# Bazs/structure_from_motion

Measured on AMD Instinct MI355X. Metric: correspondence-evals/s (matches x hypotheses), higher is better.
Workload: dtype f64 (+ conservative f16/bf16 matrix-pipe reject filter)

## Files before the change

structure_from_motion_amd/csrc/sfm_score.hip:

```cpp
#include <hip/hip_runtime.h>
#include <math.h>
#include <stdint.h>
#include <stdlib.h>

#include <algorithm>
#include <atomic>

#include "sfm_common.h"
#include "sfm_math.h"
#include "sfm_score_ws.h"
#include "sfm_score_matrix.h"

namespace {

using namespace sfmws;
using sfmhost::check_launch;
using sfmhost::fail;
using sfmhost::grid_for;
using sfmhost::grid_stride;

constexpr int kHypPerWave = 4;
#ifndef SFM_WAVE_STAMPS
#define SFM_WAVE_STAMPS 0
#endif
// ... 237 lines not shown
        c[k] = 0;
    }
    const int limit = min(n, kEstimatePoints);
    for (int i = lane; i < limit; i += kWave) {
        const float4 p = pts32[i];
#pragma unroll
        for (int k = 0; k < HPW; ++k) {
            if (ONE_SIDED) {
                const unsigned long long rej = reject_mask_one_sided(f[k], p.x, p.y, p.z, p.w);
                c[k] += (int)((~rej >> lane) & 1ull);
            } else {
                c[k] += filter_rejects(f[k], T, p.x, p.y, p.z, p.w) ? 0 : 1;
            }
        }
    }
#pragma unroll
    for (int k = 0; k < HPW; ++k) {
        const int total = sfm::wave_sum(c[k]);
        const int h = h0 + k;
        if (h < h_count && lane == 0) estimate[b * (int64_t)h_count + h] = total * 16;
    }
}

SFM_DEVICE int cost_class(int estimate) {
    if (estimate <= 0) return kClasses - 1;
    const unsigned e = (unsigned)min(estimate, 16384);
    const int lg = 31 - __builtin_clz(e);
    const int sixteenth = lg >= 4 ? (int)((e >> (lg - 4)) & 15u) : (int)((e << (4 - lg)) & 15u);
    return 16 * (14 - lg) + (15 - sixteenth);
}
static_assert(kEstimatePoints == 1024 && kClasses == 16 * 15 + 1, "cost_class: estimates up to 2^14 in 240 classes + one for zero");

__global__ __launch_bounds__(256) void score_class_count_kernel(const int32_t* __restrict__ estimate, int h_count,
                                                                int32_t* __restrict__ buckets) {
    static_assert(kClasses <= 256, "one thread per class");
    __shared__ int block_count[256];
    const int64_t b = blockIdx.y;
    const int h = blockIdx.x * blockDim.x + threadIdx.x;
    block_count[threadIdx.x] = 0;
    __syncthreads();
    if (h < h_count) atomicAdd(&block_count[cost_class(estimate[b * (int64_t)h_count + h])], 1);
    __syncthreads();
    if (threadIdx.x < kClasses && block_count[threadIdx.x] != 0)
        atomicAdd(buckets + b * kBuckets + threadIdx.x * kClassStride, block_count[threadIdx.x]);
}

__global__ __launch_bounds__(256) void score_class_scan_kernel(int32_t* __restrict__ buckets, int64_t batch) {
    __shared__ int scan[256];
    const int64_t b = blockIdx.x;
    const int c = threadIdx.x;
    const int own = c < kClasses ? buckets[b * kBuckets + c * kClassStride] : 0;
    scan[c] = own;
    __syncthreads();
#pragma unroll
// ... 435 lines not shown

void launch_matrix_setup(const sfmhost::ScorePlan& p, const sfmhost::ScoreArrays& io, unsigned* select_state) {
    hipLaunchKernelGGL(matrixscore::matrix_setup_kernel, dim3(p.matrix.setup_blocks, (unsigned)p.batch), dim3(256), 0, io.stream,
                       (const Corr*)io.corr, (int)p.n, p.a_scale, p.partial, p.buckets, io.cnt, (int)p.h_count, select_state);
}

int launch_matrix(const sfmhost::ScorePlan& p, const sfmhost::ScoreArrays& io, bool tables_ready, bool fold_in_selection) {
    using namespace matrixscore;
    static_assert(kBlocks * 2 * 16 == 96, "sfm_score_ws.h sizes the tables: 3 blocks");
    const auto& m = p.matrix;
    const unsigned pairs = (unsigned)p.batch;
    if (!tables_ready) {
        launch_matrix_setup(p, io, nullptr);
        hipLaunchKernelGGL(matrix_tables_kernel, dim3((unsigned)m.table_blocks + grid_for(2 * p.h_count, 256), pairs), dim3(256), 0,
                           io.stream, (const Corr*)io.corr, (int)p.n, p.a_scale, (const float4*)p.partial, (int)m.setup_blocks, p.table,
                           m.table_blocks, io.E, (int)p.h_count, p.hyp_table, io.S, p.thr, p.fix);
    }
    const int32_t* order_arg = nullptr;
    if (p.use_order) {
        hipLaunchKernelGGL((score_sed_matrix_kernel<true, 0, false>), dim3(m.prepass_blocks), dim3(256), 0, io.stream, (const Corr*)io.corr,
                           (const uint4*)p.hyp_table, (const uint4*)p.table, (int)p.n, io.E, (int)p.h_count, p.thr, (const int32_t*)nullptr,
                           io.cnt, io.s1, io.s2, m.prepass_units, m.prepass_steps, (unsigned char*)nullptr, (const unsigned char*)nullptr,
                           (int)p.batch, m.prepass_blocks_per_pair, (int32_t*)nullptr, p.record, p.per_unit, p.ws.units,
                           (const int32_t*)nullptr, 0);
        const dim3 per_hyp(grid_for(p.h_count, 256), pairs);
        hipLaunchKernelGGL(score_class_count_kernel, per_hyp, dim3(256), 0, io.stream, io.cnt, (int)p.h_count, p.buckets);
        hipLaunchKernelGGL(score_class_scan_scatter_kernel, per_hyp, dim3(256), 0, io.stream, io.cnt, (int)p.h_count, p.buckets, p.order,
                           m.wide_from_min, m.wide_from_max);
        const int rc = check_launch("score order kernels");
        if (rc != SFM_OK) return rc;
        order_arg = p.order;
    }
    if (p.opt.timing_before) (void)hipEventRecord((hipEvent_t)p.opt.timing_before, io.stream);
    const auto scoring_kernel = m.wide_waves ? score_sed_matrix_kernel<false, SFM_MATRIX_MASK_GROUP_WIDE, true>
                                : p.batch > 1 ? score_sed_matrix_kernel<false, SFM_MATRIX_MASK_GROUP_BATCH, false>
                                              : score_sed_matrix_kernel<false, SFM_MATRIX_MASK_GROUP_SINGLE, false>;
    hipLaunchKernelGGL(scoring_kernel, dim3(m.scoring_blocks), dim3(256), 0, io.stream, (const Corr*)io.corr, (const uint4*)p.hyp_table,
                       (const uint4*)p.table, (int)p.n, io.E, (int)p.h_count, p.thr, order_arg, io.cnt, io.s1, io.s2, p.ws.units, p.per_unit,
                       p.split, (const unsigned char*)p.fix, (int)p.batch, m.blocks_per_pair, m.persistent ? p.buckets + kTicketWords : nullptr,
                       p.record, 0, 0, m.wide_waves ? p.buckets + kWideFromWord : nullptr, m.wide_from_max);
    if (p.opt.timing_after) (void)hipEventRecord((hipEvent_t)p.opt.timing_after, io.stream);
    if (!fold_in_selection && p.ws.units > 1)
        hipLaunchKernelGGL(matrix_fold_kernel, dim3(grid_stride(p.h_count, 256, 1024), pairs), dim3(256), 0, io.stream, p.split,
                           (const unsigned char*)p.fix, p.ws.units, (int)p.h_count, io.cnt, io.s1, io.s2);
    return check_launch("score_sed_matrix_kernel");
}

constexpr sfm_score_options kBuiltinOptions = SFM_SCORE_OPTIONS_DEFAULT;
std::atomic<const sfm_score_options*> g_default_options{&kBuiltinOptions};

bool valid_options(const sfm_score_options& o) {
    return (o.kernel == SFM_SCORE_KERNEL_AUTO || o.kernel == SFM_SCORE_KERNEL_FILTERED || o.kernel == SFM_SCORE_KERNEL_MATRIX) &&
           (o.hyps_per_wave == 0 || o.hyps_per_wave == 1 || o.hyps_per_wave == 2 || o.hyps_per_wave == 4) && o.split >= -1 &&
           o.order >= -1 && o.order <= 1 && o.one_sided >= -1 && o.one_sided <= 1 && o.xcd_map >= -1 && o.xcd_map <= 1 &&
           o.block_sync >= -1 && o.persistent >= -1 && o.persistent <= 1;
}

bool load_options(const sfm_score_options* given, sfm_score_options* out) {
    *out = given ? *given : *g_default_options.load(std::memory_order_acquire);
    return valid_options(*out);
}

int refuse(const char* fn, const char* what) {
    snprintf(sfmhost::error_buffer(), sfmhost::kErrorBytes, "%s: %s", fn, what);
    return SFM_EINVAL;
}
constexpr const char* kBeyondOneLaunch = "size exceeds what one launch covers (2^31-1 blocks, 2^32-1 threads in x; 65535 in y/z)";

bool use_matrix_kernel(int64_t n, int64_t h_count, int64_t batch, const sfm_score_options& opt) {
    const int matrix_env = opt.kernel == SFM_SCORE_KERNEL_MATRIX ? 1 : opt.kernel == SFM_SCORE_KERNEL_FILTERED ? 0 : -1;
    const int64_t waves32_all = (h_count + matrixscore::kHyps - 1) / matrixscore::kHyps * batch;
    const bool matrix_fits = n <= matrixscore::kMaxPoints &&
                             sfmhost::grid_fits((int64_t)grid_for((h_count + 31) / 32, 256 / kWave) * ((batch + 7) / 8 * 8), 1, 256);
    const bool matrix_pays = batch == 1 ? (n >= 4000 && h_count >= 2048 && (double)n * (double)h_count >= 3.5e8)
                                        : (n >= 8192 && h_count >= 1024 && waves32_all >= 6144 &&
                                           (double)n * (double)h_count * (double)batch >= 5e8);
    return matrix_fits && (matrix_env > 0 || (matrix_env < 0 && matrix_pays));
}

constexpr int kRecordRangesPerWave = 2;

int plan_launches(const char* fn, sfmhost::ScorePlan* p) {
    const int64_t n = p->n, h_count = p->h_count, batch = p->batch;
    const sfm_score_options& opt = p->opt;
    int hpw = kHypPerWave;
    if (opt.hyps_per_wave != 0) {
        hpw = opt.hyps_per_wave;
    } else {
        while (hpw > 1 && (h_count + hpw - 1) / hpw * batch < 5120) hpw /= 2;
    }
    if (!sfmhost::grid_fits((h_count + hpw - 1) / hpw, 256 / kWave, 256, batch)) return refuse(fn, kBeyondOneLaunch);
    if (!sfmhost::grid_fits(h_count, 256, 256, batch)) return refuse(fn, "the ordering pre-pass exceeds what one launch covers");
    const int64_t waves = (h_count + kHypPerWave - 1) / kHypPerWave;
    const int order_env = opt.order;
    const bool use_order = order_env >= 0 ? order_env != 0 : (waves * batch <= 12 * 5120 && n >= 8192);
    const bool matrix = use_matrix_kernel(n, h_count, batch, opt);
    const bool one_sided = opt.one_sided != 0;
    p->a_scale = matrix ? matrixscore::scale_for(p->thr) : (one_sided ? one_sided_scale(p->thr) : 1.0);
    const int split_env = opt.split;
    p->small.hpw = opt.hyps_per_wave != 0 ? opt.hyps_per_wave : (h_count + 1) / 2 >= 5120 ? 2 : 1;
    p->small.blocks = grid_for((h_count + p->small.hpw - 1) / p->small.hpw, 256 / kWave);
    p->small.sync_every = opt.block_sync >= 0 ? opt.block_sync : (p->small.hpw == 1 && n >= 4096 ? 2 : 0);
    p->small.prep_blocks = (int)((n + kPrepPoints - 1) / kPrepPoints);
// ... 55 lines not shown
                        steps_per_unit >= kReplaySteps && steps - (m_units - 1) * steps_per_unit >= kReplaySteps;
    p->ws = WsPlan{true, m_units, record};
    p->use_order = matrix_order;
    p->per_unit = steps_per_unit;
    auto& m = p->matrix;
    m.setup_blocks = grid_stride(n, 1024, matrixscore::kSetupBlocks);
    m.table_blocks = (int)((matrixscore::table_steps(n) + 3) / 4);
    m.wide_waves = batch == 1 && matrix_order && h_count >= SFM_MATRIX_WIDE_MIN_HYPOTHESES;
    m.wide_from_min = m.wide_waves ? SFM_MATRIX_WIDE_FROM : 0;
    m.wide_from_max = m.wide_waves ? matrixscore::kWideFromMax : 0;
    using matrixscore::kHyps;
    const int64_t scoring_waves = m.wide_waves ? m.wide_from_max / kHyps + (h_count + 2 * kHyps - 1) / (2 * kHyps) : waves32;
    const unsigned blocks = grid_for(scoring_waves, 256 / kWave);
    const unsigned blocks_of_32 = grid_for(waves32, 256 / kWave);
    const unsigned groups = batch > 1 ? (unsigned)((batch + 7) / 8 * 8) : 1u;
    m.blocks_per_pair = batch > 1 ? (int)blocks * m_units : 0;
    m.persistent = batch == 1 && opt.persistent > 0;
    m.scoring_blocks = blocks * groups * (unsigned)m_units;
    const int e_steps = matrixscore::estimate_steps(n);
    m.prepass_units = record ? (batch == 1 ? std::max(1, m_units / kRecordRangesPerWave) : 1) : (batch == 1 && e_steps >= 128 ? 4 : 1);
    m.prepass_steps = record ? kReplaySteps : e_steps / m.prepass_units;
    m.prepass_blocks = blocks_of_32 * groups * (unsigned)m.prepass_units;
    m.prepass_blocks_per_pair = batch > 1 ? (int)blocks_of_32 * m.prepass_units : 0;
    return SFM_OK;
}

int compute_units() {
    static std::atomic<int> cached[64];
    int device = 0;
    if (hipGetDevice(&device) != hipSuccess || device < 0 || device >= 64) return 256;
    int cus = cached[device].load(std::memory_order_relaxed);
    if (cus == 0) {
        if (hipDeviceGetAttribute(&cus, hipDeviceAttributeMultiprocessorCount, device) != hipSuccess || cus <= 0) cus = 256;
        cached[device].store(cus, std::memory_order_relaxed);
    }
    return cus;
}

}

namespace sfmhost {

int plan_score(const char* fn, int64_t n, int64_t h_count, int64_t batch, double thr, const sfm_score_options* options,
               void* workspace, int64_t workspace_bytes, ScorePlan* plan) {
    *plan = ScorePlan{};
    plan->n = n;
// ... 216 lines not shown
```

structure_from_motion_amd/csrc/sfm_score_matrix.h:

```cpp
#pragma once

#ifndef SFM_MATRIX_OCC
#define SFM_MATRIX_OCC 4
#endif
#ifndef SFM_MATRIX_POPS
#define SFM_MATRIX_POPS 4
#endif
#ifndef SFM_MATRIX_MASK_GROUP_SINGLE
#define SFM_MATRIX_MASK_GROUP_SINGLE 4
#endif
#ifndef SFM_MATRIX_MASK_GROUP_WIDE
#define SFM_MATRIX_MASK_GROUP_WIDE 2
#endif
#ifndef SFM_MATRIX_MASK_GROUP_BATCH
#define SFM_MATRIX_MASK_GROUP_BATCH 2
#endif
#ifndef SFM_MATRIX_STATS
#define SFM_MATRIX_STATS 0
#endif

#include "sfm_matrix_tables.h"

namespace matrixscore {

#if SFM_MATRIX_STATS
__device__ unsigned long long g_matrix_stats[4];
// ... 17 lines not shown
#endif
constexpr int kWideOcc = 3;
#ifndef SFM_MATRIX_WIDE_MIN_HYPOTHESES
#define SFM_MATRIX_WIDE_MIN_HYPOTHESES 8192
#endif
#ifndef SFM_MATRIX_WIDE_FROM
#define SFM_MATRIX_WIDE_FROM 4096
#endif
constexpr int kWideFromMax = 4 * SFM_MATRIX_WIDE_FROM;
static_assert(kWideFromMax % kHyps == 0, "waves of 32 cover the entries [0, kWideFromMax) exactly");
constexpr int kCap = SFM_MATRIX_CAP;
constexpr int kHigh = kCap - 4;
constexpr int kLow = 8;
constexpr int kPops = SFM_MATRIX_POPS;
#ifndef SFM_MATRIX_AHEAD
#define SFM_MATRIX_AHEAD 1
#endif
static_assert(SFM_MATRIX_AHEAD >= 1 && kHigh + 2 * (SFM_MATRIX_AHEAD + 1) - 1 <= kCap, "a group of kAhead + 1 steps (two entries each in a wide wave) must fit behind kHigh - 1 entries");
static_assert(SFM_MATRIX_AHEAD + 1 <= 4, "the point operand table is padded to a multiple of four steps");
constexpr int kAhead = SFM_MATRIX_AHEAD;
#ifndef SFM_MATRIX_ESTIMATE_AHEAD
#define SFM_MATRIX_ESTIMATE_AHEAD 1
#endif
static_assert(SFM_MATRIX_ESTIMATE_AHEAD == 1 || SFM_MATRIX_ESTIMATE_AHEAD == 3, "the recording pre-pass packs steps in pairs; the table is padded to four steps");
#ifndef SFM_MATRIX_ESTIMATE_STEPS
#define SFM_MATRIX_ESTIMATE_STEPS 128
#endif
constexpr int kEstimateSteps = SFM_MATRIX_ESTIMATE_STEPS;
constexpr int64_t kMaxPoints = sfmws::kMatrixMaxPoints;
constexpr int kMaxRangeSteps = 32768;
static_assert(kMaxPoints <= (int64_t)sfmws::kSplitMaxUnits * kMaxRangeSteps * kTile, "sixteen ranges of 2^15 steps cover the largest pair");

__host__ __device__ inline int estimate_steps(int64_t n) {
    const int64_t eighth = steps_of(n) / 8;
    return (int)(eighth < 32 ? 32 : eighth > kEstimateSteps ? kEstimateSteps : eighth);
}

__global__ __launch_bounds__(256) void matrix_prepare_kernel(const Corr* __restrict__ corr, int n, double c,
                                                            const unsigned char* __restrict__ ws, uint4* __restrict__ table) {
    const int64_t pair = blockIdx.y;
    const int t = (int)blockIdx.x * 4 + (int)(threadIdx.x / kWave);
    if (t >= (int)table_steps(n)) return;
    prepare_step(corr + pair * (int64_t)n, n, c, reinterpret_cast<const uint32_t*>(ws + 16 * pair),
                 table + pair * table_steps(n) * kBlocks * 64, t, (int)(threadIdx.x & (kWave - 1)));
}

__global__ __launch_bounds__(256) void matrix_hypothesis_kernel(const unsigned char* __restrict__ ws, const double* __restrict__ E,
// ... 194 lines not shown
    const f16x8 B1 = __builtin_bit_cast(f16x8, operands[1]);
    const bf16x8 B2 = __builtin_bit_cast(bf16x8, operands[2]);
    const uint4* __restrict__ operands_second = hyp_table + ((int64_t)h_second * 2 + half) * kBlocks;
    const f16x8 C0 = __builtin_bit_cast(f16x8, operands_second[0]);
    const f16x8 C1 = __builtin_bit_cast(f16x8, operands_second[1]);
    const bf16x8 C2 = __builtin_bit_cast(bf16x8, operands_second[2]);
    SFM_STAMP(1);

    int c = 0;
    unsigned head = 0, tail = 0, cur = 0;
    constexpr unsigned kSlotBytes = kWave * 4, kRingMask = (kCap - 1) * kSlotBytes;
    typedef __attribute__((address_space(3))) uint32_t lds_u32;
    const uint32_t queue_base = (uint32_t)(uintptr_t)(lds_u32*)my_queue;
    auto ring_slot = [&](unsigned counter) __attribute__((always_inline)) {
        return (lds_u32*)(uintptr_t)(queue_base | (counter & kRingMask));
    };
    unsigned cur_off = 0;
    double a1 = 0.0, a2 = 0.0;
#if SFM_MATRIX_STATS || SFM_MATRIX_STAMPS
    unsigned stat_rounds = 0, stat_pops = 0, stat_push_iterations = 0;
#endif

    const int steps_total = (int)steps_of(n);
    const bool recording = ESTIMATE && a.record != nullptr;
    const bool replaying = !ESTIMATE && a.record != nullptr;
    const int step_begin = units > 1 ? unit * (recording ? a.range_stride : steps_per_unit) : 0;
    const int64_t record_stride = sfmws::split_padded(h_count) * 2;
    uint4* const my_record = a.record == nullptr ? nullptr
        : reinterpret_cast<uint4*>(a.record) + (int64_t)unit * (kReplaySteps / 8) * record_stride + (int64_t)h * 2 + (WIDE ? 0 : half);
    const int step_end = units > 1 || ESTIMATE ? min(step_begin + steps_per_unit, steps_total) : steps_total;
    const int last_loadable = (int)table_steps(n) - 1;

    const sfm::SedGate gate = sfm::sed_gate(thr);
    const unsigned lane_off = (unsigned)((step_begin * kTile + (WIDE ? 0 : 16 * half) - 16) * (int)sizeof(Corr));
    auto round = [&]() __attribute__((always_inline)) {
        Corr p[kPops];
        bool active[kPops];
#pragma unroll
        for (int k = 0; k < kPops; ++k) {
            if ((cur == 0u) & (head != tail)) {
                const unsigned entry = *ring_slot(head);
                head += kSlotBytes;
                cur = entry & 0xffffu;
                cur_off = lane_off + ((entry >> 16) << (WIDE ? 9 : 10));
            }
            active[k] = cur != 0u;
            const unsigned lz = (unsigned)__builtin_clz(cur | 1u);
            cur &= ~(0x80000000u >> lz);
            const unsigned off = active[k] ? cur_off + (lz << 5) : 0u;
// ... 5 lines not shown
        for (int k = 0; k < kPops; ++k) stat_pops += active[k] ? 1u : 0u;
#endif
        auto evaluate = [&](int from, int to) __attribute__((always_inline)) {
#pragma unroll
            for (int k = from; k < to; ++k) {
                double sed;
                const bool ok = sfm::sed_inlier(e, p[k].xa, p[k].ya, p[k].xb, p[k].yb, gate, sed) && active[k];
                c += ok ? 1 : 0;
                const double kept = ok ? sed : 0.0;
                a1 += kept;
                a2 = fma(kept, kept, a2);
            }
        };
        if (MASK_GROUP > 0) {
#pragma unroll
            for (int g = 0; g < kPops; g += (MASK_GROUP > 0 ? MASK_GROUP : kPops))
                if (active[g]) evaluate(g, g + MASK_GROUP < kPops ? g + MASK_GROUP : kPops);
        } else {
            evaluate(0, kPops);
        }
    };

    unsigned survivors = 0;
    unsigned rec[4] = {0u, 0u, 0u, 0u}, rec_low = 0u;
    unsigned rec_upper[4] = {0u, 0u, 0u, 0u}, rec_upper_low = 0u;
    static_assert((kAhead + 1) % 2 == 0, "the recording pre-pass packs the steps of a loop group two to a dword");
    const int first_step = step_begin + (replaying ? kReplaySteps : 0);
    if (step_begin < step_end) {
        const uint4* __restrict__ src = table + lane;
        const unsigned lane_bytes = (unsigned)lane * 16u;
        const __amdgpu_buffer_rsrc_t table_rsrc = __builtin_amdgcn_make_buffer_rsrc(
            const_cast<uint4*>(table), (short)0, (int)(table_steps(n) * (int64_t)(kBlocks * 64 * 16)), 0x00020000);
        constexpr int kStages = (ESTIMATE ? SFM_MATRIX_ESTIMATE_AHEAD : kAhead) + 1;
        uint4 A[kStages][kBlocks];
#pragma unroll
        for (int a = 0; a < kStages; ++a) {
#pragma unroll
            for (int b = 0; b < kBlocks; ++b) A[a][b] = src[((size_t)min(first_step + a, last_loadable) * kBlocks + b) * 64];
            __builtin_amdgcn_sched_barrier(0);
        }
        if (replaying) {
            unsigned words[kReplaySteps / 2], words_upper[kReplaySteps / 2];
#pragma unroll
            for (int q = 0; q < kReplaySteps / 8; ++q) {
                const uint4 w = my_record[q * record_stride];
                words[4 * q] = w.x, words[4 * q + 1] = w.y, words[4 * q + 2] = w.z, words[4 * q + 3] = w.w;
                if (WIDE) {
                    const uint4 u = my_record[q * record_stride + 1];
                    words_upper[4 * q] = u.x, words_upper[4 * q + 1] = u.y, words_upper[4 * q + 2] = u.z, words_upper[4 * q + 3] = u.w;
// ... 40 lines not shown
                float16v r2 = {0, 0, 0, 0, 0, 0, 0, 0, 0, 0, 0, 0, 0, 0, 0, 0}, d2 = r2;
                r2 = __builtin_amdgcn_mfma_f32_32x32x16_f16(__builtin_bit_cast(f16x8, A[stage][0]), C0, r2, 0, 0, 0);
                d2 = __builtin_amdgcn_mfma_f32_32x32x16_bf16(__builtin_bit_cast(bf16x8, A[stage][2]), C2, d2, 0, 0, 0);
                r2 = __builtin_amdgcn_mfma_f32_32x32x16_f16(__builtin_bit_cast(f16x8, A[stage][1]), C1, r2, 0, 0, 0);
                unsigned second = 0;
#pragma unroll
                for (int j = 0; j < 16; ++j)
                    second = __builtin_amdgcn_alignbit(second, __float_as_uint(__builtin_fmaf(-r2[j], r2[j], d2[j])), 31);
                const auto swapped = __builtin_amdgcn_permlane32_swap(rejected, second, false, false);
                rejected = swapped[0];
                rejected_upper = swapped[1];
            }
#define SFM_KEEP_OF(REJECTED) (~(REJECTED) & 0xffffu)
            {
                unsigned step_bytes = (unsigned)min(t + kStages, last_loadable) * (unsigned)(kBlocks * 64 * 16);
                asm volatile("" : "+s"(step_bytes), "+v"(rejected), "+v"(rejected_upper));
#pragma unroll
                for (int b = 0; b < kBlocks; ++b)
                    A[stage][b] = __builtin_bit_cast(uint4, __builtin_amdgcn_raw_buffer_load_b128(table_rsrc, (int)lane_bytes + b * 1024, (int)step_bytes, 0));
            }
            if (ESTIMATE) {
                survivors += (unsigned)__builtin_popcount(SFM_KEEP_OF(rejected));
                if (WIDE) survivors += (unsigned)__builtin_popcount(SFM_KEEP_OF(rejected_upper));
                if (recording) {
                    if (stage & 1) {
                        rec[0] = rec[1];
                        rec[1] = rec[2];
                        rec[2] = rec[3];
                        rec[3] = rec_low | (rejected << 16);
                        if (WIDE) {
                            rec_upper[0] = rec_upper[1];
                            rec_upper[1] = rec_upper[2];
                            rec_upper[2] = rec_upper[3];
                            rec_upper[3] = rec_upper_low | (rejected_upper << 16);
                        }
                    } else {
                        rec_low = rejected;
                        rec_upper_low = rejected_upper;
                    }
                }
            } else {
                const unsigned field = WIDE ? 2u * (unsigned)(t - step_begin) : (unsigned)(t - step_begin);
                if (rejected != 0xffffu) {
                    *ring_slot(tail) = ~(rejected ^ ((field << 16) ^ 0xffff0000u));
                    tail += kSlotBytes;
                }
                if (WIDE && rejected_upper != 0xffffu) {
                    *ring_slot(tail) = ~(rejected_upper ^ (((field + 1u) << 16) ^ 0xffff0000u));
                    tail += kSlotBytes;
                }
            }
          }
          t0 += kStages;
          if (recording && ((t0 - step_begin) & 7) == 0)
          {
              my_record[((t0 - step_begin) / 8 - 1) * record_stride] = make_uint4(rec[0], rec[1], rec[2], rec[3]);
              if (WIDE) my_record[((t0 - step_begin) / 8 - 1) * record_stride + 1] = make_uint4(rec_upper[0], rec_upper[1], rec_upper[2], rec_upper[3]);
          }
          queue_full = !ESTIMATE && __builtin_amdgcn_ballot_w64((int)(tail - head) >= kHigh * (int)kSlotBytes) != 0ull;
         } while (t0 < step_end && !queue_full);
         if (queue_full) {
             __builtin_amdgcn_wave_barrier();
             do round(); while (__builtin_amdgcn_ballot_w64((int)(tail - head) > kLow * (int)kSlotBytes) != 0ull);
         }
        }
    }
    if (ESTIMATE) {
        const unsigned both = WIDE ? survivors : survivors + (unsigned)__shfl_xor((int)survivors, 32, 64);
        const unsigned scanned = (unsigned)min(units * steps_per_unit * kTile, n);
        unsigned sixteenths = (unsigned)(((unsigned long long)both * 16384ull) / (scanned > 0u ? scanned : 1u));
        sixteenths = both > 0u && sixteenths == 0u ? 1u : sixteenths;
        if ((WIDE || half == 0) && valid) {
            if (units > 1) atomicAdd(cnt + h, (int32_t)sixteenths);
            else cnt[h] = (int32_t)sixteenths;
        }
        return;
    }
    SFM_STAMP(2);
    __builtin_amdgcn_wave_barrier();
    while (__builtin_amdgcn_ballot_w64(tail != head || cur != 0u) != 0ull) round();
    SFM_STAMP(3);
// ... 29 lines not shown
        }
    }
#if SFM_MATRIX_STAMPS
    SFM_STAMP(5);
    const unsigned wave_id = item_id;
    if (lane == 0 && wave_id < 65536u) {
        unsigned hw_id;
        asm volatile("s_getreg_b32 %0, hwreg(HW_REG_HW_ID)" : "=s"(hw_id));
        unsigned xcc_id;
        asm volatile("s_getreg_b32 %0, hwreg(HW_REG_XCC_ID)" : "=s"(xcc_id));
#pragma unroll
        for (int k = 0; k < 6; ++k) g_matrix_stamps[10 * wave_id + k] = stamp[k];
        g_matrix_stamps[10 * wave_id + 6] = ((unsigned long long)xcc_id << 32) | hw_id;
        g_matrix_stamps[10 * wave_id + 7] = ((unsigned long long)unit << 32) | (unsigned)h0;
        g_matrix_stamps[10 * wave_id + 9] = __builtin_amdgcn_s_memtime() - clock_begin;
    }
    {
        unsigned long long pops = stat_pops;
#pragma unroll
        for (int off = 32; off > 0; off >>= 1) pops += __shfl_xor((unsigned)pops, off, 64);
        if (lane == 0 && wave_id < 65536u) g_matrix_stamps[10 * wave_id + 8] = ((unsigned long long)stat_rounds << 32) | (unsigned)pops;
    }
#endif
}

__global__ __launch_bounds__(256) void matrix_fold_kernel(const unsigned char* __restrict__ split, const unsigned char* __restrict__ fix,
                                                          int units, int h_count, int32_t* __restrict__ cnt,
                                                          double* __restrict__ s1, double* __restrict__ s2) {
    const int64_t pair = blockIdx.y;
    const int64_t hp = sfmws::split_padded(h_count);
    split += pair * sfmws::split_bytes(h_count, units);
    if (fix != nullptr) fix += pair * sfmws::matrix_fix_bytes(h_count);
    cnt += pair * (int64_t)h_count;
    s1 += pair * (int64_t)h_count;
    s2 += pair * (int64_t)h_count;
    const int32_t* part_c = reinterpret_cast<const int32_t*>(split) + hp;
    const double* part_a1 = reinterpret_cast<const double*>(part_c + (int64_t)units * hp);
    const double* part_a2 = part_a1 + (int64_t)units * hp;
    const int32_t* fix_c = reinterpret_cast<const int32_t*>(fix);
    const double* fix_a1 = reinterpret_cast<const double*>(fix + 4 * hp);
    for (int64_t h = (int64_t)blockIdx.x * blockDim.x + threadIdx.x; h < h_count; h += (int64_t)gridDim.x * blockDim.x) {
        int total = part_c[h];
        double t1 = part_a1[h], t2 = part_a2[h];
        for (int u = 1; u < units; ++u) {
            total += part_c[u * hp + h];
            t1 += part_a1[u * hp + h];
            t2 += part_a2[u * hp + h];
        }
        if (fix != nullptr) {
            total += fix_c[h];
            t1 += fix_a1[h];
            t2 += fix_a1[hp + h];
        }
        cnt[h] = total;
        s1[h] = t1;
        s2[h] = t2;
    }
}

template <bool ESTIMATE, int MASK_GROUP = 0, bool WIDE_WAVES = false>
__global__ __launch_bounds__(256, WIDE_WAVES ? kWideOcc : SFM_MATRIX_OCC) void score_sed_matrix_kernel(
    const Corr* __restrict__ pts, const uint4* __restrict__ hyp_table, const uint4* __restrict__ table, int n,
    const double* __restrict__ E, int h_count, double thr, const int32_t* __restrict__ order, int32_t* __restrict__ cnt,
    double* __restrict__ s1, double* __restrict__ s2, int units, int steps_per_unit, unsigned char* __restrict__ split,
    const unsigned char* __restrict__ fix, int batch, int blocks_per_pair, int32_t* __restrict__ tickets,
    uint16_t* __restrict__ record, int range_stride, int record_ranges, const int32_t* __restrict__ wide_word, int wide_max) {
    __shared__ alignas(kCap * kWave * 4) uint32_t queues[ESTIMATE ? 1 : 256 / kWave][ESTIMATE ? 1 : kCap][kWave];
    const int lane = threadIdx.x & (kWave - 1);
    const int wave_in_block = __builtin_amdgcn_readfirstlane((int)(threadIdx.x / kWave));
    uint32_t* const my_queue = &queues[ESTIMATE ? 0 : wave_in_block][0][lane];
    MatrixPair a{pts, hyp_table, table, E, order, cnt, s1, s2, split, fix, record, range_stride};
    int wide_from = WIDE_WAVES ? (wide_word != nullptr ? min(*wide_word, h_count) : 0) : h_count;
    const int narrow_waves = wide_max / kHyps;
    auto item = [&](int wave, int unit, unsigned item_id, int ranges) __attribute__((always_inline)) {
        if (WIDE_WAVES && wave >= narrow_waves)
            matrix_item<ESTIMATE, MASK_GROUP, true>(a, n, h_count, thr, ranges, steps_per_unit, wide_from + (wave - narrow_waves) * 2 * kHyps, h_count,
                                                    unit, my_queue, lane, item_id);
        else
            matrix_item<ESTIMATE, MASK_GROUP, false>(a, n, h_count, thr, ranges, steps_per_unit, wave * kHyps, wide_from, unit, my_queue, lane,
                                                     item_id);
    };
    if (tickets != nullptr) {
        const int waves32 = WIDE_WAVES ? narrow_waves + (h_count - wide_from + 2 * kHyps - 1) / (2 * kHyps) : (h_count + kHyps - 1) / kHyps;
        const bool by_xcc = units % 8 == 0;
        unsigned xcc = 0;
        if (by_xcc) {
            asm volatile("s_getreg_b32 %0, hwreg(HW_REG_XCC_ID)" : "=s"(xcc));
            xcc &= 7u;
        }
        const int mine = by_xcc ? units / 8 : units;
        const int items = waves32 * mine;
        for (unsigned k = 0; k < (by_xcc ? 8u : 1u); ++k) {
            const unsigned x = (xcc + k) & 7u;
            for (;;) {
                const int t = take_ticket(tickets + 16 * x);
                if (t >= items) break;
                const int wave = t / mine;
                const int unit = by_xcc ? (int)x + 8 * (t % mine) : t % mine;
                item(wave, unit, (unsigned)(wave * units + unit), units);
            }
        }
        return;
    }
    int block_of_range = blockIdx.x, unit = 0;
    if (batch > 1) {
// ... 3 lines not shown
        if (pair >= batch) return;
        if (units > 1) {
            unit = block_of_range % units;
            block_of_range /= units;
            if (a.split != nullptr) a.split += pair * sfmws::split_bytes(h_count, units);
        }
        a.pts += pair * (int64_t)n;
        a.table += pair * table_steps(n) * kBlocks * 64;
        a.hyp_table += pair * (int64_t)h_count * 2 * kBlocks;
        a.E += pair * (int64_t)h_count * 9;
        if (a.order != nullptr) a.order += pair * (int64_t)h_count;
        a.cnt += pair * (int64_t)h_count;
        a.s1 += pair * (int64_t)h_count;
        a.s2 += pair * (int64_t)h_count;
        if (a.fix != nullptr) a.fix += pair * sfmws::matrix_fix_bytes(h_count);
        if (a.record != nullptr) a.record += pair * (sfmws::matrix_record_bytes(h_count) / 2);
        if (WIDE_WAVES && wide_word != nullptr) wide_from = min(wide_word[pair * sfmws::kBuckets], h_count);
    } else if (units > 1) {
        unit = block_of_range % units;
        block_of_range /= units;
    }
    const int wave = block_of_range * (256 / kWave) + wave_in_block;
    if (ESTIMATE && record != nullptr) {
        const int per_wave = record_ranges / units;
        for (int p = 0; p < per_wave; ++p)
            item(wave, unit * per_wave + p, 0u, record_ranges);
        return;
    }
    item(wave, unit, blockIdx.x * (256 / kWave) + wave_in_block, units);
}

}
```

structure_from_motion_amd/csrc/sfm_score_ws.h:

```cpp
#pragma once
#include <hip/hip_runtime.h>
#include <stdint.h>

#include "sfm_common.h"

namespace sfmws {

constexpr int kEstimatePoints = 1024;
constexpr int kClasses = 16 * 15 + 1;
constexpr int kClassStride = 16;
constexpr int kBuckets = 256 * kClassStride;
constexpr int64_t kPointsPad = 4096;

constexpr int kPrepPoints = 512;
constexpr int kSmallMaxPoints = 8192;
constexpr int kMaxPrepBlocks = kSmallMaxPoints / kPrepPoints;
static_assert(4 * kMaxPrepBlocks <= kBuckets, "the partial maxima live in the class-counter words");
constexpr int kFusedShards = 32;
constexpr int kFusedPartialOffset = 64;

__host__ __device__ inline int64_t ws_points_offset(int64_t batch) { return 16 * batch; }
__host__ __device__ inline int64_t ws_buckets_offset(int64_t n, int64_t batch) {
    return 16 * batch + 16 * n * batch + kPointsPad;
}
// ... 14 lines not shown
    return split_padded(h_count) * (4 + (int64_t)(units > 1 ? units : 0) * (4 + 8 + 8));
}
__host__ __device__ inline int64_t split_region_bytes(int64_t h_count, int64_t batch, int units) {
    return batch == 1 ? split_bytes(h_count, units) : (units > 1 ? batch * split_bytes(h_count, units) : 0);
}
constexpr int64_t kMatrixMaxPoints = 1 << 22;
__host__ __device__ inline int64_t matrix_table_steps(int64_t n) { return (((n + 31) / 32) + 3) & ~(int64_t)3; }
__host__ __device__ inline int64_t matrix_table_bytes(int64_t n) { return matrix_table_steps(n) * 3 * 64 * 16; }
__host__ __device__ inline int64_t matrix_hyp_table_bytes(int64_t h_count) { return h_count * 96; }
__host__ __device__ inline int64_t matrix_fix_bytes(int64_t h_count) { return split_padded(h_count) * (4 + 8 + 8); }
__host__ __device__ inline int64_t ws_matrix_offset(int64_t n, int64_t h_count, int64_t batch, const WsPlan& plan) {
    return ((ws_tail_offset(n, h_count, batch) + split_region_bytes(h_count, batch, plan.units) + 255) / 256) * 256;
}
__host__ __device__ inline int64_t ws_matrix_hyp_offset(int64_t n, int64_t h_count, int64_t batch, const WsPlan& plan) {
    return ((ws_matrix_offset(n, h_count, batch, plan) + (plan.matrix ? batch * matrix_table_bytes(n) : 0) + 255) / 256) * 256;
}
__host__ __device__ inline int64_t ws_matrix_fix_offset(int64_t n, int64_t h_count, int64_t batch, const WsPlan& plan) {
    return ((ws_matrix_hyp_offset(n, h_count, batch, plan) + (plan.matrix ? batch * matrix_hyp_table_bytes(h_count) : 0) + 255) / 256) * 256;
}
#ifndef SFM_MATRIX_ESTIMATE_STEPS
#define SFM_MATRIX_ESTIMATE_STEPS 128
#endif
constexpr int kMatrixReplaySteps = 16;
__host__ __device__ inline int64_t matrix_record_bytes(int64_t h_count) {
    return split_padded(h_count) * (int64_t)((SFM_MATRIX_ESTIMATE_STEPS / kMatrixReplaySteps) * (kMatrixReplaySteps / 8) * 2 * 16);
}
__host__ __device__ inline int64_t ws_matrix_record_offset(int64_t n, int64_t h_count, int64_t batch, const WsPlan& plan) {
    return ((ws_matrix_fix_offset(n, h_count, batch, plan) + (plan.matrix ? batch * matrix_fix_bytes(h_count) : 0) + 255) / 256) * 256;
}
__host__ __device__ inline int64_t workspace_bytes_for(int64_t n, int64_t h_count, int64_t batch, const WsPlan& plan) {
    return ws_matrix_record_offset(n, h_count, batch, plan) + (plan.record ? matrix_record_bytes(h_count) : 0);
}
constexpr int kWideFromWord = 3844;
constexpr int kTicketWords = 3968;
constexpr int kTicketWordsPrepass = 3848;
static_assert(16 * (kClasses - 1) < kWideFromWord && kWideFromWord < kTicketWordsPrepass, "a free word behind the class counters");
static_assert(16 * (kClasses - 1) < kTicketWordsPrepass && kTicketWordsPrepass + 8 * 8 <= kTicketWords &&
              kTicketWords + 8 * 16 <= kBuckets, "the work counters sit between the class counters and the end of the block");

__device__ __forceinline__ float4 to_filter_point(const Corr& p, double a_scale) {
    return make_float4((float)(p.xa * a_scale), (float)(p.ya * a_scale), (float)p.xb, (float)p.yb);
}

__device__ __forceinline__ void prepare_small_block(const Corr* __restrict__ pts, int n, double a_scale,
                                                    unsigned char* __restrict__ ws, int block) {
    const int lane = threadIdx.x & (kWave - 1);
    float4* __restrict__ out = reinterpret_cast<float4*>(ws + ws_points_offset(1));
    int32_t* buckets = reinterpret_cast<int32_t*>(ws + ws_buckets_offset(n, 1));
    Corr p[8];
    const int base = block * kPrepPoints + lane;
#pragma unroll
    for (int j = 0; j < 8; ++j) p[j] = pts[min(base + j * kWave, n - 1)];
    float m0 = 0.f, m1 = 0.f, m2 = 0.f, m3 = 0.f;
#pragma unroll
    for (int j = 0; j < 8; ++j) {
        const int i = base + j * kWave;
        if (i < n) {
            const float4 q = to_filter_point(p[j], a_scale);
            out[i] = q;
            m0 = fmaxf(m0, fabsf(q.x));
            m1 = fmaxf(m1, fabsf(q.y));
// ... 37 lines not shown
    int32_t* order;
    unsigned char* split;
    float4* partial;
    uint4* table;
    uint4* hyp_table;
    unsigned char* fix;
    uint16_t* record;
    struct {
        int hpw;
        bool one_sided;
        unsigned prepare_blocks;
        unsigned blocks;
        int blocks_per_pair;
        dim3 scoring_grid;
    } valu;
    struct {
        unsigned setup_blocks;
        int table_blocks;
        bool wide_waves;
        int wide_from_min, wide_from_max;
        int prepass_units, prepass_steps;
        unsigned prepass_blocks;
        int prepass_blocks_per_pair;
        bool persistent;
        unsigned scoring_blocks;
        int blocks_per_pair;
    } matrix;
    struct {
        int hpw, sync_every;
        unsigned blocks;
        int prep_blocks;
        double a_scale;
        int32_t* order;
    } small;
    int deferred_units() const { return ws.matrix ? ws.units : 1; }
};

struct ScoreArrays {
    const double* corr;
    const double* E;
    const int32_t* S;
    int32_t* cnt;
    double* s1;
    double* s2;
    hipStream_t stream;
};
// ... 10 lines not shown
```

Baseline: 4656 billion.

## Dedicated software-pipelined recording prepass with optional fused class counting

Replaces the generic matrix_item path used for the recording estimate prepass with a specialized prepass_record_wave routine. It multi-buffers raw buffer loads of the point table across stages, runs the MFMA reject filter, and packs reject masks into the record table. It also converts survivor counts into sixteenth estimates atomically. It raises the prepass occupancy bound and optionally folds cost-class counting into the prepass, off by default, to drop a separate kernel. The cost is more specialized code and register pressure from staged operands.

```diff
diff --git a/structure_from_motion_amd/csrc/sfm_score.hip b/structure_from_motion_amd/csrc/sfm_score.hip
--- a/structure_from_motion_amd/csrc/sfm_score.hip
+++ b/structure_from_motion_amd/csrc/sfm_score.hip
@@ -283,14 +283,6 @@
     }
 }
 
-SFM_DEVICE int cost_class(int estimate) {
-    if (estimate <= 0) return kClasses - 1;
-    const unsigned e = (unsigned)min(estimate, 16384);
-    const int lg = 31 - __builtin_clz(e);
-    const int sixteenth = lg >= 4 ? (int)((e >> (lg - 4)) & 15u) : (int)((e << (4 - lg)) & 15u);
-    return 16 * (14 - lg) + (15 - sixteenth);
-}
-static_assert(kEstimatePoints == 1024 && kClasses == 16 * 15 + 1, "cost_class: estimates up to 2^14 in 240 classes + one for zero");
 
 __global__ __launch_bounds__(256) void score_class_count_kernel(const int32_t* __restrict__ estimate, int h_count,
                                                                 int32_t* __restrict__ buckets) {
@@ -772,9 +764,10 @@
                            (const uint4*)p.hyp_table, (const uint4*)p.table, (int)p.n, io.E, (int)p.h_count, p.thr, (const int32_t*)nullptr,
                            io.cnt, io.s1, io.s2, m.prepass_units, m.prepass_steps, (unsigned char*)nullptr, (const unsigned char*)nullptr,
                            (int)p.batch, m.prepass_blocks_per_pair, (int32_t*)nullptr, p.record, p.per_unit, p.ws.units,
-                           (const int32_t*)nullptr, 0);
+                           (const int32_t*)nullptr, 0, m.prepass_counts_classes ? p.buckets : (int32_t*)nullptr);
         const dim3 per_hyp(grid_for(p.h_count, 256), pairs);
-        hipLaunchKernelGGL(score_class_count_kernel, per_hyp, dim3(256), 0, io.stream, io.cnt, (int)p.h_count, p.buckets);
+        if (!m.prepass_counts_classes)
+            hipLaunchKernelGGL(score_class_count_kernel, per_hyp, dim3(256), 0, io.stream, io.cnt, (int)p.h_count, p.buckets);
         hipLaunchKernelGGL(score_class_scan_scatter_kernel, per_hyp, dim3(256), 0, io.stream, io.cnt, (int)p.h_count, p.buckets, p.order,
                            m.wide_from_min, m.wide_from_max);
         const int rc = check_launch("score order kernels");
@@ -788,7 +781,7 @@
     hipLaunchKernelGGL(scoring_kernel, dim3(m.scoring_blocks), dim3(256), 0, io.stream, (const Corr*)io.corr, (const uint4*)p.hyp_table,
                        (const uint4*)p.table, (int)p.n, io.E, (int)p.h_count, p.thr, order_arg, io.cnt, io.s1, io.s2, p.ws.units, p.per_unit,
                        p.split, (const unsigned char*)p.fix, (int)p.batch, m.blocks_per_pair, m.persistent ? p.buckets + kTicketWords : nullptr,
-                       p.record, 0, 0, m.wide_waves ? p.buckets + kWideFromWord : nullptr, m.wide_from_max);
+                       p.record, 0, 0, m.wide_waves ? p.buckets + kWideFromWord : nullptr, m.wide_from_max, (int32_t*)nullptr);
     if (p.opt.timing_after) (void)hipEventRecord((hipEvent_t)p.opt.timing_after, io.stream);
     if (!fold_in_selection && p.ws.units > 1)
         hipLaunchKernelGGL(matrix_fold_kernel, dim3(grid_stride(p.h_count, 256, 1024), pairs), dim3(256), 0, io.stream, p.split,
@@ -827,8 +820,6 @@
                                            (double)n * (double)h_count * (double)batch >= 5e8);
     return matrix_fits && (matrix_env > 0 || (matrix_env < 0 && matrix_pays));
 }
-
-constexpr int kRecordRangesPerWave = 2;
 
 int plan_launches(const char* fn, sfmhost::ScorePlan* p) {
     const int64_t n = p->n, h_count = p->h_count, batch = p->batch;
@@ -930,6 +921,7 @@
     m.prepass_steps = record ? kReplaySteps : e_steps / m.prepass_units;
     m.prepass_blocks = blocks_of_32 * groups * (unsigned)m.prepass_units;
     m.prepass_blocks_per_pair = batch > 1 ? (int)blocks_of_32 * m.prepass_units : 0;
+    m.prepass_counts_classes = record && SFM_MATRIX_PREPASS_CLASSES != 0;
     return SFM_OK;
 }
 
diff --git a/structure_from_motion_amd/csrc/sfm_score_matrix.h b/structure_from_motion_amd/csrc/sfm_score_matrix.h
--- a/structure_from_motion_amd/csrc/sfm_score_matrix.h
+++ b/structure_from_motion_amd/csrc/sfm_score_matrix.h
@@ -2,6 +2,15 @@
 
 #ifndef SFM_MATRIX_OCC
 #define SFM_MATRIX_OCC 4
+#endif
+#ifndef SFM_MATRIX_PREPASS_OCC
+#define SFM_MATRIX_PREPASS_OCC 5
+#endif
+#ifndef SFM_MATRIX_PREPASS_STAGES
+#define SFM_MATRIX_PREPASS_STAGES 2
+#endif
+#ifndef SFM_MATRIX_PREPASS_CLASSES
+#define SFM_MATRIX_PREPASS_CLASSES 0
 #endif
 #ifndef SFM_MATRIX_POPS
 #define SFM_MATRIX_POPS 4
@@ -65,7 +74,7 @@
 #ifndef SFM_MATRIX_ESTIMATE_AHEAD
 #define SFM_MATRIX_ESTIMATE_AHEAD 1
 #endif
-static_assert(SFM_MATRIX_ESTIMATE_AHEAD == 1 || SFM_MATRIX_ESTIMATE_AHEAD == 3, "the recording pre-pass packs steps in pairs; the table is padded to four steps");
+static_assert(SFM_MATRIX_ESTIMATE_AHEAD == 1 || SFM_MATRIX_ESTIMATE_AHEAD == 3, "the point operand table is padded to a multiple of four steps");
 #ifndef SFM_MATRIX_ESTIMATE_STEPS
 #define SFM_MATRIX_ESTIMATE_STEPS 128
 #endif
@@ -306,9 +315,8 @@
 #endif
 
     const int steps_total = (int)steps_of(n);
-    const bool recording = ESTIMATE && a.record != nullptr;
     const bool replaying = !ESTIMATE && a.record != nullptr;
-    const int step_begin = units > 1 ? unit * (recording ? a.range_stride : steps_per_unit) : 0;
+    const int step_begin = units > 1 ? unit * steps_per_unit : 0;
     const int64_t record_stride = sfmws::split_padded(h_count) * 2;
     uint4* const my_record = a.record == nullptr ? nullptr
         : reinterpret_cast<uint4*>(a.record) + (int64_t)unit * (kReplaySteps / 8) * record_stride + (int64_t)h * 2 + (WIDE ? 0 : half);
@@ -360,9 +368,6 @@
     };
 
     unsigned survivors = 0;
-    unsigned rec[4] = {0u, 0u, 0u, 0u}, rec_low = 0u;
-    unsigned rec_upper[4] = {0u, 0u, 0u, 0u}, rec_upper_low = 0u;
-    static_assert((kAhead + 1) % 2 == 0, "the recording pre-pass packs the steps of a loop group two to a dword");
     const int first_step = step_begin + (replaying ? kReplaySteps : 0);
     if (step_begin < step_end) {
         const uint4* __restrict__ src = table + lane;
@@ -449,23 +454,6 @@
             if (ESTIMATE) {
                 survivors += (unsigned)__builtin_popcount(SFM_KEEP_OF(rejected));
                 if (WIDE) survivors += (unsigned)__builtin_popcount(SFM_KEEP_OF(rejected_upper));
-                if (recording) {
-                    if (stage & 1) {
-                        rec[0] = rec[1];
-                        rec[1] = rec[2];
-                        rec[2] = rec[3];
-                        rec[3] = rec_low | (rejected << 16);
-                        if (WIDE) {
-                            rec_upper[0] = rec_upper[1];
-                            rec_upper[1] = rec_upper[2];
-                            rec_upper[2] = rec_upper[3];
-                            rec_upper[3] = rec_upper_low | (rejected_upper << 16);
-                        }
-                    } else {
-                        rec_low = rejected;
-                        rec_upper_low = rejected_upper;
-                    }
-                }
             } else {
                 const unsigned field = WIDE ? 2u * (unsigned)(t - step_begin) : (unsigned)(t - step_begin);
                 if (rejected != 0xffffu) {
@@ -479,11 +467,6 @@
             }
           }
           t0 += kStages;
-          if (recording && ((t0 - step_begin) & 7) == 0)
-          {
-              my_record[((t0 - step_begin) / 8 - 1) * record_stride] = make_uint4(rec[0], rec[1], rec[2], rec[3]);
-              if (WIDE) my_record[((t0 - step_begin) / 8 - 1) * record_stride + 1] = make_uint4(rec_upper[0], rec_upper[1], rec_upper[2], rec_upper[3]);
-          }
           queue_full = !ESTIMATE && __builtin_amdgcn_ballot_w64((int)(tail - head) >= kHigh * (int)kSlotBytes) != 0ull;
          } while (t0 < step_end && !queue_full);
          if (queue_full) {
@@ -559,6 +542,114 @@
         if (lane == 0 && wave_id < 65536u) g_matrix_stamps[10 * wave_id + 8] = ((unsigned long long)stat_rounds << 32) | (unsigned)pops;
     }
 #endif
+}
+
+constexpr int kLastTag = 1 << 24;
+static_assert(sfmws::kSplitMaxUnits * kLastTag > 0 && 16384 < kLastTag, "estimates and the count of contributions share a word");
+template <int STAGES, int RANGES>
+SFM_DEVICE void prepass_record_wave(const MatrixPair& a, int n, int h_count, int ranges, int first_range, int wave, int lane,
+                                    int32_t* __restrict__ classes) {
+    static_assert(STAGES >= 2 && STAGES <= 4 && kReplaySteps % 8 == 0, "the table is padded to four steps; whole 16-byte chunks");
+    const int h0 = wave * kHyps;
+    if (h0 >= h_count) return;
+    const int col = lane & 31, half = lane >> 5;
+    const int h = min(h0 + col, h_count - 1);
+    const bool owner = half == 0 && h0 + col < h_count;
+    const uint4* __restrict__ operands = a.hyp_table + ((int64_t)h * 2 + half) * kBlocks;
+    const f16x8 B0 = __builtin_bit_cast(f16x8, operands[0]);
+    const f16x8 B1 = __builtin_bit_cast(f16x8, operands[1]);
+    const bf16x8 B2 = __builtin_bit_cast(bf16x8, operands[2]);
+    const int last_loadable = (int)table_steps(n) - 1;
+    const unsigned lane_bytes = (unsigned)lane * 16u;
+    const __amdgpu_buffer_rsrc_t table_rsrc = __builtin_amdgcn_make_buffer_rsrc(
+        const_cast<uint4*>(a.table), (short)0, (int)(table_steps(n) * (int64_t)(kBlocks * 64 * 16)), 0x00020000);
+    uint4 A[STAGES][kBlocks];
+    auto load_stage = [&](int stage, unsigned step_bytes) __attribute__((always_inline)) {
+#pragma unroll
+        for (int b = 0; b < kBlocks; ++b)
+            A[stage][b] = __builtin_bit_cast(uint4, __builtin_amdgcn_raw_buffer_load_b128(table_rsrc, (int)lane_bytes, (int)step_bytes + b * 1024, 0));
+    };
+    constexpr unsigned kStepBytes = kBlocks * 64 * 16;
+#pragma unroll
+    for (int s = 0; s < STAGES; ++s) {
+        load_stage(s, (unsigned)min(first_range * a.range_stride + s, last_loadable) * kStepBytes);
+        __builtin_amdgcn_sched_barrier(0);
+    }
+    const int64_t record_stride = sfmws::split_padded(h_count) * 2;
+    const unsigned record_off = (unsigned)(h * 2 + half) * 16u, cnt_off = (unsigned)h * 4u;
+    auto my_cnt = [&]() __attribute__((always_inline)) {
+        unsigned off = cnt_off;
+        asm volatile("" : "+v"(off));
+        return reinterpret_cast<int32_t*>(reinterpret_cast<unsigned char*>(a.cnt) + off);
+    };
+    const unsigned scanned = (unsigned)min(ranges * kReplaySteps * kTile, n);
+    constexpr bool kCountClasses = SFM_MATRIX_PREPASS_CLASSES != 0;
+
+    auto count_class = [&](int returned, unsigned contributed) __attribute__((always_inline)) {
+        const bool last = owner && (returned >> 24) == ranges - 1;
+        int cls = 0;
+        if (last) {
+            atomicAdd(my_cnt(), -ranges * kLastTag);
+            cls = sfmws::cost_class((returned & (kLastTag - 1)) + (int)contributed);
+        }
+        unsigned long long todo = __builtin_amdgcn_ballot_w64(last);
+        while (todo != 0ull) {
+            const int leader = __builtin_ctzll(todo);
+            const int leader_class = __builtin_amdgcn_readlane(cls, leader);
+            const unsigned long long same = __builtin_amdgcn_ballot_w64(last && cls == leader_class);
+            if (lane == leader) atomicAdd(classes + leader_class * sfmws::kClassStride, (int32_t)__builtin_popcountll(same));
+            todo &= ~same;
+        }
+    };
+
+    int returned = 0;
+    unsigned contributed = 0u;
+#pragma unroll
+    for (int p = 0; p < RANGES; ++p) {
+        unsigned char* const chunk = reinterpret_cast<unsigned char*>(reinterpret_cast<uint4*>(a.record) + (int64_t)(first_range + p) * (kReplaySteps / 8) * record_stride);
+        unsigned words[4], rejects = 0u;
+#pragma unroll
+        for (int s = 0; s < kReplaySteps; ++s) {
+            const int stage = (p * kReplaySteps + s) % STAGES;
+            float16v r = {0, 0, 0, 0, 0, 0, 0, 0, 0, 0, 0, 0, 0, 0, 0, 0}, d = r;
+            r = __builtin_amdgcn_mfma_f32_32x32x16_f16(__builtin_bit_cast(f16x8, A[stage][0]), B0, r, 0, 0, 0);
+            d = __builtin_amdgcn_mfma_f32_32x32x16_bf16(__builtin_bit_cast(bf16x8, A[stage][2]), B2, d, 0, 0, 0);
+            r = __builtin_amdgcn_mfma_f32_32x32x16_f16(__builtin_bit_cast(f16x8, A[stage][1]), B1, r, 0, 0, 0);
+            unsigned rejected = 0;
+#pragma unroll
+            for (int j = 0; j < 16; ++j)
+                rejected = __builtin_amdgcn_alignbit(rejected, __float_as_uint(__builtin_fmaf(-r[j], r[j], d[j])), 31);
+            const int ahead = p * kReplaySteps + s + STAGES;
+            if (ahead < RANGES * kReplaySteps) {
+                unsigned step_bytes = (unsigned)min((first_range + ahead / kReplaySteps) * a.range_stride + ahead % kReplaySteps, last_loadable) * kStepBytes;
+                asm volatile("" : "+s"(step_bytes), "+v"(rejected));
+                load_stage(stage, step_bytes);
+            }
+            __builtin_amdgcn_sched_barrier(0);
+            if (s & 1) words[(s >> 1) & 3] |= rejected << 16;
+            else words[(s >> 1) & 3] = rejected;
+            if ((s & 7) == 7) {
+                unsigned chunk_off = record_off;
+                asm volatile("" : "+v"(chunk_off));
+                *reinterpret_cast<uint4*>(chunk + (s >> 3) * record_stride * 16 + chunk_off) = make_uint4(words[0], words[1], words[2], words[3]);
+#pragma unroll
+                for (int k = 0; k < 4; ++k) rejects += (unsigned)__builtin_popcount(words[k]);
+            }
+        }
+        const unsigned survivors = 16u * kReplaySteps - rejects;
+        const unsigned both = survivors + (unsigned)__shfl_xor((int)survivors, 32, 64);
+        unsigned sixteenths = (both * 16384u) / (scanned > 0u ? scanned : 1u);
+        sixteenths = both > 0u && sixteenths == 0u ? 1u : sixteenths;
+        if (!kCountClasses) {
+            if (owner) atomicAdd(my_cnt(), (int32_t)sixteenths);
+        } else {
+            if (p > 0) count_class(returned, contributed);
+            returned = owner ? atomicAdd(my_cnt(), (int32_t)sixteenths + kLastTag) : 0;
+            contributed = sixteenths;
+        }
+        __builtin_amdgcn_sched_barrier(0);
+    }
+    if (kCountClasses) count_class(returned, contributed);
 }
 
 __global__ __launch_bounds__(256) void matrix_fold_kernel(const unsigned char* __restrict__ split, const unsigned char* __restrict__ fix,
@@ -596,12 +687,13 @@
 }
 
 template <bool ESTIMATE, int MASK_GROUP = 0, bool WIDE_WAVES = false>
-__global__ __launch_bounds__(256, WIDE_WAVES ? kWideOcc : SFM_MATRIX_OCC) void score_sed_matrix_kernel(
+__global__ __launch_bounds__(256, ESTIMATE ? SFM_MATRIX_PREPASS_OCC : WIDE_WAVES ? kWideOcc : SFM_MATRIX_OCC) void score_sed_matrix_kernel(
     const Corr* __restrict__ pts, const uint4* __restrict__ hyp_table, const uint4* __restrict__ table, int n,
     const double* __restrict__ E, int h_count, double thr, const int32_t* __restrict__ order, int32_t* __restrict__ cnt,
     double* __restrict__ s1, double* __restrict__ s2, int units, int steps_per_unit, unsigned char* __restrict__ split,
     const unsigned char* __restrict__ fix, int batch, int blocks_per_pair, int32_t* __restrict__ tickets,
-    uint16_t* __restrict__ record, int range_stride, int record_ranges, const int32_t* __restrict__ wide_word, int wide_max) {
+    uint16_t* __restrict__ record, int range_stride, int record_ranges, const int32_t* __restrict__ wide_word, int wide_max,
+    int32_t* __restrict__ classes) {
     __shared__ alignas(kCap * kWave * 4) uint32_t queues[ESTIMATE ? 1 : 256 / kWave][ESTIMATE ? 1 : kCap][kWave];
     const int lane = threadIdx.x & (kWave - 1);
     const int wave_in_block = __builtin_amdgcn_readfirstlane((int)(threadIdx.x / kWave));
@@ -617,7 +709,7 @@
             matrix_item<ESTIMATE, MASK_GROUP, false>(a, n, h_count, thr, ranges, steps_per_unit, wave * kHyps, wide_from, unit, my_queue, lane,
                                                      item_id);
     };
-    if (tickets != nullptr) {
+    if (!ESTIMATE && tickets != nullptr) {
         const int waves32 = WIDE_WAVES ? narrow_waves + (h_count - wide_from + 2 * kHyps - 1) / (2 * kHyps) : (h_count + kHyps - 1) / kHyps;
         const bool by_xcc = units % 8 == 0;
         unsigned xcc = 0;
@@ -667,9 +759,8 @@
     }
     const int wave = block_of_range * (256 / kWave) + wave_in_block;
     if (ESTIMATE && record != nullptr) {
-        const int per_wave = record_ranges / units;
-        for (int p = 0; p < per_wave; ++p)
-            item(wave, unit * per_wave + p, 0u, record_ranges);
+        prepass_record_wave<SFM_MATRIX_PREPASS_STAGES, sfmws::kRecordRangesPerWave>(a, n, h_count, record_ranges,
+                                                                                   unit * sfmws::kRecordRangesPerWave, wave, lane, classes);
         return;
     }
     item(wave, unit, blockIdx.x * (256 / kWave) + wave_in_block, units);
diff --git a/structure_from_motion_amd/csrc/sfm_score_ws.h b/structure_from_motion_amd/csrc/sfm_score_ws.h
--- a/structure_from_motion_amd/csrc/sfm_score_ws.h
+++ b/structure_from_motion_amd/csrc/sfm_score_ws.h
@@ -60,6 +60,7 @@
 #define SFM_MATRIX_ESTIMATE_STEPS 128
 #endif
 constexpr int kMatrixReplaySteps = 16;
+constexpr int kRecordRangesPerWave = 2;
 __host__ __device__ inline int64_t matrix_record_bytes(int64_t h_count) {
     return split_padded(h_count) * (int64_t)((SFM_MATRIX_ESTIMATE_STEPS / kMatrixReplaySteps) * (kMatrixReplaySteps / 8) * 2 * 16);
 }
@@ -75,6 +76,15 @@
 static_assert(16 * (kClasses - 1) < kWideFromWord && kWideFromWord < kTicketWordsPrepass, "a free word behind the class counters");
 static_assert(16 * (kClasses - 1) < kTicketWordsPrepass && kTicketWordsPrepass + 8 * 8 <= kTicketWords &&
               kTicketWords + 8 * 16 <= kBuckets, "the work counters sit between the class counters and the end of the block");
+
+__device__ __forceinline__ int cost_class(int estimate) {
+    if (estimate <= 0) return kClasses - 1;
+    const unsigned e = (unsigned)min(estimate, 16384);
+    const int lg = 31 - __builtin_clz(e);
+    const int sixteenth = lg >= 4 ? (int)((e >> (lg - 4)) & 15u) : (int)((e << (4 - lg)) & 15u);
+    return 16 * (14 - lg) + (15 - sixteenth);
+}
+static_assert(kEstimatePoints == 1024 && kClasses == 16 * 15 + 1, "cost_class: estimates up to 2^14 in 240 classes + one for zero");
 
 __device__ __forceinline__ float4 to_filter_point(const Corr& p, double a_scale) {
     return make_float4((float)(p.xa * a_scale), (float)(p.ya * a_scale), (float)p.xb, (float)p.yb);
@@ -158,6 +168,7 @@
         int prepass_units, prepass_steps;
         unsigned prepass_blocks;
         int prepass_blocks_per_pair;
+        bool prepass_counts_classes;
         bool persistent;
         unsigned scoring_blocks;
         int blocks_per_pair;
```

Result: no change. 4670 billion, median of 6 (+0.3%).
